# vt-asaplab/porla

Measured on AMD Instinct MI355X. Metric: BN254 G1 MSM Mscalar-mul/s at 2^20 pts, higher is better.
Workload: dtype u32x8 (256-bit modular integer); 1 GPU; KZG scheme, single 2^20-point BN254 G1 MSM per GPU, inputs resident in HBM, output 64-B affine point; pairs_per_gpu=1048576, msm_in_flight=2, warmup_steps_run=41, collective=none (single GPU)

## Files before the change

porla_amd/csrc/ec30.hip.h:

```cpp
#pragma once
#include "ec.hip.h"
#include "fe30.hip.h"

namespace porla {

template <class M>
struct XYZZ30 {
    F30<M> x, y, zz, zzz;
    bool inf;
};

template <class M>
__device__ __forceinline__ XYZZ<M> xyzz30_to_xyzz(const XYZZ30<M>& p);

template <class M>
__device__ __noinline__ XYZZ30<M> xyzz30_double_affine(F30<M> ax, F30<M> ay) {
    XYZZ30<M> r;
    F30<M> U = f30_small_mul<M, 2>(ay);
    F30<M> V = f30_sqr<M>(U);
    F30<M> W = f30_mul<M>(U, V);
    F30<M> S = f30_mul<M>(ax, V);
    F30<M> XX = f30_sqr<M>(ax);
    F30<M> Mm = f30_small_mul<M, 3>(XX);
    F30<M> MM = f30_sqr<M>(Mm);
// ... 210 lines not shown
    }
    xyzz30_add<M>(a, b);
    xyzz30_store_lazy<M>(p, a);
}
template <class M>
__device__ __noinline__ void xyzz30_double_mem(XYZZ<M>* p, int times) {
    XYZZ30<M> a = xyzz30_load_lazy<M>(p);
    if (a.inf) return;
#pragma unroll 1
    for (int t = 0; t < times && !a.inf; t++) a = xyzz30_double_body<M>(a.x, a.y, a.zz, a.zzz);
    xyzz30_store_lazy<M>(p, a);
}

template <int CTRL>
__device__ __forceinline__ uint32_t dpp_quad(uint32_t v) {
    return (uint32_t)__builtin_amdgcn_update_dpp(0, (int)v, CTRL, 0xf, 0xf, true);
}
template <class M, int CTRL>
__device__ __forceinline__ F30<M> f30_quad(const F30<M>& a) {
    F30<M> r;
#pragma unroll
    for (int i = 0; i < 9; i++) r.v[i] = dpp_quad<CTRL>(a.v[i]);
    return r;
}
template <class M>
__device__ __forceinline__ F30<M> f30_sel(bool c, const F30<M>& a, const F30<M>& b) {
    F30<M> r;
#pragma unroll
    for (int i = 0; i < 9; i++) r.v[i] = c ? a.v[i] : b.v[i];
    return r;
}
template <class M>
__device__ __forceinline__ F30<M> xyzz30_load_coord(const XYZZ<M>* p, int c, bool* all_zero) {
    const uint4* q = reinterpret_cast<const uint4*>(reinterpret_cast<const uint32_t*>(p) + 8 * c);
    const uint4 a = q[0], b = q[1];
    uint32_t t[8] = {a.x, a.y, a.z, a.w, b.x, b.y, b.z, b.w};
    *all_zero = (a.x | a.y | a.z | a.w | b.x | b.y | b.z | b.w) == 0;
    return f30_unpack<M>(t);
}
template <class M>
__device__ __forceinline__ void xyzz30_store_coord(XYZZ<M>* p, int c, const F30<M>& v, bool final) {
    uint32_t* d = reinterpret_cast<uint32_t*>(p) + 8 * c;
    Fe<M> t;
    if (final) {
        t = f30_to_fe_canonical<M>(f30_mul<M>(v, f30_const<M>(M::R1)));
    } else if constexpr (M::PSEUDO_MERSENNE) {
        t = f30_to_fe_canonical<M>(f30_pm_reduce<M>(v));
    } else {
        f30_pack<M>(t.v, v);
    }
    store_words8(d, t.v);
}
template <class M>
__device__ __noinline__ void xyzz30_add_one_lane(const XYZZ<M>* pa, const XYZZ<M>* pb, XYZZ<M>* out, bool final) {
    XYZZ30<M> a = xyzz30_load_lazy<M>(pa), b = xyzz30_load_lazy<M>(pb);
    xyzz30_add<M>(a, b);
    if (final) {
        const XYZZ<M> r = xyzz30_to_xyzz<M>(a);
        uint32_t* d = reinterpret_cast<uint32_t*>(out);
        store_words8(d, r.x.v); store_words8(d + 8, r.y.v); store_words8(d + 16, r.zz.v); store_words8(d + 24, r.zzz.v);
    } else {
        xyzz30_store_lazy<M>(out, a);
    }
}
template <class M>
__device__ __forceinline__ void xyzz30_add_quad(const XYZZ<M>* pa, const XYZZ<M>* pb, XYZZ<M>* out, bool final, bool live,
                                                uint32_t lane) {
    const uint32_t r = lane & 3u;
    const XYZZ<M>* sa = (r & 1u) ? pb : pa;
    const XYZZ<M>* sb = (r & 1u) ? pa : pb;
    bool za, zb;
    const F30<M> A = xyzz30_load_coord<M>(sa, (int)(r >> 1), &za);
    const F30<M> B = xyzz30_load_coord<M>(sb, 2 + (int)(r >> 1), &zb);
    bool special = zb;
    if (!final) {
        const uint32_t qz = (uint32_t)(__ballot(zb) >> (lane & 60u)) & 0xfu;
        if (qz) {
            const XYZZ<M>* src = (qz & 0x5u) ? pa : pb;
            if (live && src != out) {
                const uint4* q = reinterpret_cast<const uint4*>(reinterpret_cast<const uint32_t*>(src) + 8 * r);
                uint4* d = reinterpret_cast<uint4*>(reinterpret_cast<uint32_t*>(out) + 8 * r);
                const uint4 v0 = q[0], v1 = q[1];
                d[0] = v0; d[1] = v1;
            }
            return;
        }
    }
    const F30<M> M1 = f30_mul<M>(A, B);
    const bool edge = (r == 0u) || (r == 3u);
    const F30<M> rcv = f30_quad<M, 0xB1>(f30_sel<M>(edge, B, M1));
    const F30<M> D = f30_sub<M, 2>(f30_sel<M>(r == 0u, rcv, M1), f30_sel<M>(r == 0u, M1, rcv));
    const F30<M> M2 = f30_mul<M>(f30_sel<M>(edge, D, B), f30_sel<M>(edge, D, rcv));
    if (r == 0u && f30_product_is_zero<M>(M2)) special = true;
    const unsigned long long bal = __ballot(special);
    if ((bal >> (lane & 60u)) & 0xfull) {
        if (r == 0u && live) xyzz30_add_one_lane<M>(pa, pb, out, final);
        return;
    }
    const F30<M> bPP = f30_quad<M, 0x00>(M2);
    const F30<M> bU1 = f30_quad<M, 0x00>(M1);
    const F30<M> M3 = f30_mul<M>(r == 0u ? D : (r == 3u ? bU1 : M2), r == 0u ? M2 : bPP);
    const F30<M> bPPP = f30_quad<M, 0x00>(M3);
    const F30<M> bS1 = f30_quad<M, 0xAA>(M1);
    const F30<M> E = f30_add2<M>(bPPP, M3);
    const F30<M> X3 = f30_sub<M, 4>(M2, E);
    const F30<M> Dq = f30_sub<M, 6>(M3, X3);
    const F30<M> M4 = f30_mul<M>(r == 0u ? bS1 : (r == 3u ? D : M2), r == 3u ? Dq : bPPP);
    const F30<M> bT2 = f30_quad<M, 0x00>(M4);
    const F30<M> Y3 = f30_sub<M, 2>(M4, bT2);
    if (!live) return;
    if (r == 3u) { xyzz30_store_coord<M>(out, 0, X3, final); xyzz30_store_coord<M>(out, 1, Y3, final); }
    else if (r == 1u) xyzz30_store_coord<M>(out, 2, M3, final);
    else if (r == 2u) xyzz30_store_coord<M>(out, 3, M4, final);
}

template <class M>
__device__ __forceinline__ void xyzz30_dbl_quad(const XYZZ<M>* p, XYZZ<M>* out, bool live, uint32_t lane) {
    const uint32_t r = lane & 3u;
    bool zero;
    const F30<M> A = xyzz30_load_coord<M>(p, (int)r, &zero);
    const uint32_t qz = (uint32_t)(__ballot(zero && r == 2u) >> (lane & 60u)) & 0xfu;
    if (qz) {
        if (live && out != p) {
            uint4* d = reinterpret_cast<uint4*>(reinterpret_cast<uint32_t*>(out) + 8 * r);
            d[0] = make_uint4(0, 0, 0, 0); d[1] = d[0];
        }
        return;
    }
    const F30<M> U = f30_small_mul<M, 2>(A);
    const F30<M> O1 = f30_sel<M>(r == 1u, U, A);
    const F30<M> M1 = f30_mul<M>(O1, O1);
    const F30<M> bV = f30_quad<M, 0x55>(M1);
    const F30<M> bXX = f30_quad<M, 0x00>(M1);
    const F30<M> Mm = f30_small_mul<M, 3>(bXX);
    const F30<M> M2 = f30_mul<M>(r == 3u ? Mm : O1, r == 3u ? Mm : bV);
    const F30<M> bW = f30_quad<M, 0x55>(M2);
    const F30<M> bMM = f30_quad<M, 0xFF>(M2);
    const F30<M> S2 = f30_small_mul<M, 2>(M2);
    const F30<M> X3 = f30_sub<M, 3>(bMM, S2);
    const F30<M> D = f30_sub<M, 5>(M2, X3);
    const F30<M> M3 = f30_mul<M>(r == 0u ? Mm : bW, r == 0u ? D : A);
    const F30<M> bT2 = f30_quad<M, 0x55>(M3);
    const F30<M> Y3 = f30_sub<M, 2>(M3, bT2);
    if (!live) return;
    if (r == 0u) { xyzz30_store_coord<M>(out, 0, X3, false); xyzz30_store_coord<M>(out, 1, Y3, false); }
    else if (r == 2u) xyzz30_store_coord<M>(out, 2, M2, false);
    else if (r == 3u) xyzz30_store_coord<M>(out, 3, M3, false);
}

// ... 79 lines not shown
```

porla_amd/csrc/engine.hpp:

```cpp
#pragma once
#include <hip/hip_runtime.h>
#include <cstddef>
#include <cstdint>
#include <mutex>
#include <string>
#include <utility>
#include <vector>
#include "../../include/porla_gpu.h"
#include "host_curve.hpp"
#include "msm.hip.h"
#include "msm_small.hip.h"

namespace porla {

void set_last_error(const std::string& s);
int hip_fail(hipError_t e, const char* what, const char* file, int line);

#define PORLA_HIP(call)                                                      \
    do {                                                                     \
        hipError_t _e = (call);                                              \
        if (_e != hipSuccess) return ::porla::hip_fail(_e, #call, __FILE__, __LINE__); \
    } while (0)

struct ProfScope {
// ... 122 lines not shown
    void release() {
        if (h) retired.emplace_back(h, upload);
        for (auto& rb : retired) {
            if (rb.second) {
                (void)hipEventSynchronize(rb.second);
                (void)hipEventDestroy(rb.second);
            }
            (void)hipHostFree(rb.first);
        }
        retired.clear();
        h = nullptr;
        cap = 0;
        upload = nullptr;
    }
};

struct Workspace {
    std::mutex mu;
    int device = -1;
    Buf pts, keys, entries, counts, starts, fill, cursor, buckets, in_scalars, in_points;
    Buf order, blk_hist, blk_off, tile_off, heavy, chunk_out;
    Buf small_part;
    uint32_t small_seq = 0;
    Buf tree_s, tree_m, tree_mt;
    Buf multi_acc;
    hipEvent_t merged = nullptr;
    void* h_windows = nullptr;
    size_t h_windows_cap = 0;
    hipStream_t own_stream = nullptr;
    hipStream_t aux_stream = nullptr;
    hipEvent_t fork_ev = nullptr, join_ev = nullptr;
    hipEvent_t front_fork_ev = nullptr, front_join_ev = nullptr;
    hipEvent_t caller_ev = nullptr;
    int slot = 0;
    hipEvent_t done = nullptr;
    int pend_W = 0, pend_c = 0;
    bool lone = false;
    bool pair_pending = false;
    bool begun = false;
    Buf batch_list, batch_part, batch_sums, batch_ctrl, batch_out;
    PinnedList batch_list_h;
    UseFence batch_fence;
};
constexpr int MSM_SLOTS = 17;
constexpr int MSM_POOL_SLOTS = 8;
constexpr int MSM_AUDIT_SLOT = 16;
constexpr int MSM_USER_SLOTS = 4;
constexpr int MSM_MULTI_SLOT0 = 4;
constexpr int MSM_MULTI_SLOTS = 4;
constexpr int MSM_POOL_SLOT0 = 8;
int order_after_caller(Workspace* ws, hipStream_t caller, hipStream_t a, hipStream_t b = nullptr);
constexpr size_t MSM_SCAN_MAX = 1u << 16;
constexpr size_t MSM_RANGE_MAX = 1u << 22;
template <class C>
struct FixedBase {
    int device = -1;
    int c = 0, W = 0;
    size_t n_points = 0;
    Affine<typename C::Fp>* table = nullptr;
    size_t table_cap = 0;
    XYZZ<typename C::Fp>* pow_buf = nullptr;
    size_t pow_cap = 0;
    XYZZ<typename C::Fp>* scratch_buf = nullptr;
    size_t scratch_cap = 0;
    bool keep_build_buffers = false;
    XYZZ<typename C::Fp>* partial = nullptr;
    size_t partial_cap = 0;
    uint8_t* io_rows = nullptr;
    size_t io_rows_cap = 0;
    uint8_t* io_out = nullptr;
    size_t io_out_cap = 0;
    hipStream_t io_stream2 = nullptr;
    uint32_t last_S = 1;
    UseFence fence;
    static constexpr size_t HOST_FINISH_MAX_ROWS = 256;
    void* h_small = nullptr;
    void* d_small = nullptr;
    uint32_t small_seq = 0;
    hipEvent_t small_done = nullptr;
    std::mutex mu;
    void release();
    int build(const Affine<typename C::Fp>* d_base, size_t n, int window_bits, hipStream_t stream);
    int build_from_host_bytes(const uint8_t* points_be, size_t n, int window_bits, hipStream_t stream);
    int commit_device(const uint8_t* d_rows, size_t n_rows, size_t n_coeffs, size_t row_stride, uint8_t* d_out,
                      hipStream_t stream, bool guest_room = false);
    int commit_host(const uint8_t* rows, size_t n_rows, size_t n_coeffs, size_t row_stride, uint8_t* out,
                    hipStream_t stream);
    int commit_small(const uint8_t* const* row_ptrs, size_t n_rows, size_t n_coeffs, uint8_t* const* outs, hipStream_t stream,
                     const uint8_t* d_rows = nullptr, XYZZ<typename C::Fp>* raw_sums = nullptr);
    static bool small_ok(size_t n_rows, size_t n_coeffs);
};

}
struct porla_fixed_base {
    int curve;
    porla::FixedBase<porla::Bn254G1> bn;
    porla::FixedBase<porla::Secp256k1G> secp;
};
namespace porla {

extern std::mutex g_ws_mu;
extern int g_window_override;
extern int g_small_mode;
extern int g_small_c;
extern int g_last_multi[2];
extern int g_last_shape[3];
// ... 38 lines not shown
```

porla_amd/csrc/msm.hip.h:

```cpp
#pragma once
#include "ec.hip.h"
#include "ec30.hip.h"
#include "glv.hip.h"
#include <type_traits>

namespace porla {

struct Bn254G1 {
    using Fp = Bn254Fp;
    static constexpr uint32_t ORDER[8] = {0xf0000001u, 0x43e1f593u, 0x79b97091u, 0x2833e848u,
                                          0x8181585du, 0xb85045b6u, 0xe131a029u, 0x30644e72u};
    static constexpr int SCALAR_BITS = 254;
    static constexpr int MAX_Q = 5;
    using Glv = GlvBn254;
    static constexpr bool GLV_DEFAULT = false;
    static constexpr size_t GLV_BELOW = (size_t)1 << 17;
    static constexpr bool F30_BUCKETS = true;
    static constexpr bool F30_LAZY = true;
    static constexpr int BUCKET_SUM_WAVES = 4;
    static constexpr int FB_COMMIT_WAVES = 3;
    static constexpr int MACQ_WAVES = 4;
};
struct Secp256k1G {
    using Fp = Secp256k1Fp;
    static constexpr uint32_t ORDER[8] = {0xd0364141u, 0xbfd25e8cu, 0xaf48a03bu, 0xbaaedce6u,
                                          0xfffffffeu, 0xffffffffu, 0xffffffffu, 0xffffffffu};
    static constexpr int SCALAR_BITS = 256;
    static constexpr int MAX_Q = 1;
    using Glv = GlvSecp256k1;
    static constexpr bool GLV_DEFAULT = true;
    static constexpr size_t GLV_BELOW = 0;
    static constexpr bool F30_BUCKETS = true;
    static constexpr bool F30_LAZY = true;
    static constexpr int BUCKET_SUM_WAVES = 3;
    static constexpr int FB_COMMIT_WAVES = 2;
    static constexpr int MACQ_WAVES = 2;
};

constexpr uint32_t KEY_NONE = 0xffffffffu;

__device__ __forceinline__ void load_be256(uint32_t t[8], const uint8_t* p) {
    const uint4* q = reinterpret_cast<const uint4*>(p);
    uint4 hi = q[0], lo = q[1];
    t[7] = __builtin_bswap32(hi.x); t[6] = __builtin_bswap32(hi.y);
    t[5] = __builtin_bswap32(hi.z); t[4] = __builtin_bswap32(hi.w);
    t[3] = __builtin_bswap32(lo.x); t[2] = __builtin_bswap32(lo.y);
    t[1] = __builtin_bswap32(lo.z); t[0] = __builtin_bswap32(lo.w);
}
__device__ __forceinline__ void store_be256(uint8_t* p, const uint32_t t[8]) {
    uint4 hi, lo;
    hi.x = __builtin_bswap32(t[7]); hi.y = __builtin_bswap32(t[6]);
    hi.z = __builtin_bswap32(t[5]); hi.w = __builtin_bswap32(t[4]);
    lo.x = __builtin_bswap32(t[3]); lo.y = __builtin_bswap32(t[2]);
    lo.z = __builtin_bswap32(t[1]); lo.w = __builtin_bswap32(t[0]);
    uint4* q = reinterpret_cast<uint4*>(p);
    q[0] = hi; q[1] = lo;
}

template <class M>
__device__ __forceinline__ Affine<M> load_affine(const Affine<M>* pts, uint32_t idx) {
    const uint4* q = reinterpret_cast<const uint4*>(pts + idx);
    uint4 a = q[0], b = q[1], c = q[2], d = q[3];
    Affine<M> r;
    r.x.v[0] = a.x; r.x.v[1] = a.y; r.x.v[2] = a.z; r.x.v[3] = a.w;
    r.x.v[4] = b.x; r.x.v[5] = b.y; r.x.v[6] = b.z; r.x.v[7] = b.w;
    r.y.v[0] = c.x; r.y.v[1] = c.y; r.y.v[2] = c.z; r.y.v[3] = c.w;
    r.y.v[4] = d.x; r.y.v[5] = d.y; r.y.v[6] = d.z; r.y.v[7] = d.w;
    return r;
}
template <class M>
__device__ __forceinline__ void store_fe(uint32_t* dst, const Fe<M>& f) {
    uint4* q = reinterpret_cast<uint4*>(dst);
    q[0] = make_uint4(f.v[0], f.v[1], f.v[2], f.v[3]);
    q[1] = make_uint4(f.v[4], f.v[5], f.v[6], f.v[7]);
}
template <class M>
__device__ __forceinline__ Fe<M> load_fe(const uint32_t* src) {
    const uint4* q = reinterpret_cast<const uint4*>(src);
    uint4 a = q[0], b = q[1];
    Fe<M> f;
    f.v[0] = a.x; f.v[1] = a.y; f.v[2] = a.z; f.v[3] = a.w;
    f.v[4] = b.x; f.v[5] = b.y; f.v[6] = b.z; f.v[7] = b.w;
    return f;
}
template <class M>
__device__ __forceinline__ void store_xyzz(XYZZ<M>* dst, const XYZZ<M>& p) {
    uint32_t* d = reinterpret_cast<uint32_t*>(dst);
// ... 89 lines not shown
    const size_t n_sub = glv ? 2 * n : n;
    pl.tile_cap = glv ? 2 * TILE : TILE;
    pl.T_tiles = (uint32_t)((n + TILE - 1) / TILE);
    pl.lowbits = sort_lowbits(c, n_sub, W);
    pl.sort_half = false;
    {
        const int lb2 = pl.lowbits - 1, parts_log = c - 1 - lb2;
        if (lb2 >= 0 && lb2 <= 11 && parts_log <= 7 && (n_sub >> parts_log) <= 16384 && (pl.tile_cap >> parts_log) >= 64) {
            pl.lowbits = lb2;
            pl.sort_half = true;
        }
    }
    pl.P = 1 << (c - 1 - pl.lowbits);
    pl.wg = pl.T_tiles < 256 ? 256u / pl.T_tiles : 1u;
    if (pl.wg > 16) pl.wg = 16;
    if (pl.wg > (unsigned)W) pl.wg = (unsigned)W;
    return pl;
}
constexpr int SORT_HOLD_TILES = 16;
static inline bool sort_holds_runs(const SortFrontPlan& pl) { return pl.T_tiles <= 16u * SORT_HOLD_TILES; }

__device__ __forceinline__ uint32_t block_scan_1024(uint32_t v, uint32_t* wsum , uint32_t* total) {
    const uint32_t lane = threadIdx.x & 63, wv = threadIdx.x >> 6;
    uint32_t incl = v;
#pragma unroll
    for (int d = 1; d < 64; d <<= 1) {
        uint32_t o = __shfl_up(incl, d, 64);
        if (lane >= (uint32_t)d) incl += o;
    }
    if (lane == 63) wsum[wv] = incl;
    __syncthreads();
    uint32_t base = 0, tot = 0;
#pragma unroll
    for (int k = 0; k < 16; k++) {
        uint32_t s = wsum[k];
        if ((uint32_t)k < wv) base += s;
        tot += s;
    }
    __syncthreads();
    *total = tot;
    return base + incl - v;
}

template <class C, bool GLV>
__global__ void __launch_bounds__(TILE_THREADS)
k_digits_partition(const uint8_t* __restrict__ scalars, uint32_t n, int c, int W, int lowbits,
                   uint32_t* __restrict__ tile_items, uint16_t* __restrict__ tile_off, uint32_t* __restrict__ ctrl) {
    constexpr int SUBS = GLV ? 2 : 1;
    constexpr int LIMBS = GLV ? 4 : 8;
    constexpr int NSUB = TILE_SPT * SUBS;
    __shared__ uint32_t hist[MAX_PARTS];
    __shared__ uint32_t cursor[MAX_PARTS];
    __shared__ uint32_t stage[TILE * SUBS];
    const uint32_t tile = blockIdx.x, T = gridDim.x, tid = threadIdx.x;
    if (tile == 0 && blockIdx.y == 0 && tid < 4 + 128) ctrl[tid] = 0;
    const int P = 1 << (c - 1 - lowbits);
    const uint32_t B = 1u << (c - 1);
    const uint32_t mask = (1u << c) - 1;
    uint32_t t[NSUB][LIMBS];
    bool valid[TILE_SPT];
    uint32_t sneg = 0;
#pragma unroll
    for (int j = 0; j < TILE_SPT; j++) {
        uint32_t i = tile * TILE + j * TILE_THREADS + tid;
        valid[j] = i < n;
        uint32_t k[8];
#pragma unroll
        for (int q = 0; q < 8; q++) k[q] = 0;
        if (valid[j]) {
            load_be256(k, scalars + (size_t)i * 32);
            for (int q = 0; q < C::MAX_Q; q++) {
                uint32_t s[8];
                uint32_t br = 0;
#pragma unroll
                for (int q2 = 0; q2 < 8; q2++) s[q2] = sbb32(k[q2], C::ORDER[q2], br);
                if (br) break;
#pragma unroll
                for (int q2 = 0; q2 < 8; q2++) k[q2] = s[q2];
            }
        }
        if (GLV) {
            uint32_t m1[4], m2[4];
            bool n1, n2;
            glv_split<typename C::Glv>(k, m1, n1, m2, n2);
#pragma unroll
            for (int q = 0; q < 4; q++) { t[j * SUBS][q] = m1[q]; t[j * SUBS + (SUBS - 1)][q] = m2[q]; }
            sneg |= (n1 ? 1u : 0u) << (j * SUBS);
            sneg |= (n2 ? 1u : 0u) << (j * SUBS + (SUBS - 1));
        } else {
#pragma unroll
            for (int q = 0; q < LIMBS; q++) t[j][q] = k[q];
        }
    }
    uint32_t carry = 0;

    const bool shared_tile = gridDim.y > 1;
    for (int w = 0; w < W; w++) {
        const bool mine = !shared_tile || (uint32_t)w % gridDim.y == blockIdx.y;
        if (mine) {
            if (tid < MAX_PARTS) hist[tid] = 0;
            __syncthreads();
        }
        uint32_t key[NSUB];
        const int lo = w * c;
        const int limb = lo >> 5, sh = lo & 31;
        uint32_t wa[NSUB], wb[NSUB];
// ... 32 lines not shown
            if (mine && key[u] != KEY_NONE) {
                key[u] |= (dneg ^ ((sneg >> u) & 1u)) << 31;
                atomicAdd(&hist[(key[u] & 0x7fffffffu) & (uint32_t)(P - 1)], 1u);
            }
        }
        if (!mine) continue;
        __syncthreads();
        uint32_t pv = 0, pincl = 0;
        if (tid < MAX_PARTS) {
            pv = (tid < (uint32_t)P) ? hist[tid] : 0;
            pincl = pv;
#pragma unroll
            for (int d = 1; d < 64; d <<= 1) {
                const uint32_t o = __shfl_up(pincl, d, 64);
                if ((tid & 63u) >= (uint32_t)d) pincl += o;
            }
            if (tid == 63) cursor[0] = pincl;
        }
        __syncthreads();
        uint16_t* off = tile_off + ((size_t)w * T + tile) * (MAX_PARTS + 1);
        if (tid < MAX_PARTS) {
            const uint32_t excl = (tid >= 64 ? cursor[0] : 0u) + pincl - pv;
            off[tid] = (uint16_t)excl;
            hist[tid] = excl;
            if (tid == MAX_PARTS - 1) { off[MAX_PARTS] = (uint16_t)(excl + pv); cursor[1] = excl + pv; }
        }
        __syncthreads();
        const uint32_t total = cursor[1];
#pragma unroll
        for (int u = 0; u < NSUB; u++) {
            if (key[u] != KEY_NONE) {
                uint32_t bkt = key[u] & 0x7fffffffu;
                uint32_t pos = atomicAdd(&hist[bkt & (uint32_t)(P - 1)], 1u);
                uint32_t local = (uint32_t)((u / SUBS) * TILE_THREADS + tid) * SUBS + (u % SUBS);
                stage[pos] = (bkt >> (c - 1 - lowbits)) | ((key[u] >> 31) << lowbits) | (local << (lowbits + 1));
            }
        }
        __syncthreads();
        uint32_t* dst = tile_items + ((size_t)w * T + tile) * (TILE * SUBS);
        for (uint32_t i = tid; i < total; i += TILE_THREADS) dst[i] = stage[i];
        __syncthreads();
    }
}

template <int STAGE_CAP, int MAX_LOW, bool HOLD>
__global__ void __launch_bounds__(1024)
k_partition_sort(const uint32_t* __restrict__ tile_items, const uint16_t* __restrict__ tile_off, uint32_t T, uint32_t tile_cap,
                 int c, int lowbits, uint32_t* __restrict__ counts, uint32_t* __restrict__ starts,
                 uint32_t* __restrict__ entries, uint32_t* __restrict__ cursor) {
    __shared__ uint32_t cnt[MAX_LOW];
    __shared__ uint32_t stage[STAGE_CAP];
    __shared__ uint32_t wsum[16];
    __shared__ uint32_t base_sh, total_sh;
    const int P = 1 << (c - 1 - lowbits);
    const uint32_t nlow = 1u << lowbits;
    const uint32_t w = blockIdx.x / P, p = blockIdx.x % P;
    const uint32_t tid = threadIdx.x, lane = tid & 63;
    const uint32_t wv = HOLD ? (uint32_t)__builtin_amdgcn_readfirstlane((int)(tid >> 6)) : tid >> 6;
    const uint32_t lowmask = nlow - 1;
    for (uint32_t i = tid; i < nlow; i += 1024) cnt[i] = 0;
    __syncthreads();
    auto run_bounds = [&](uint32_t t, uint32_t& lo, uint32_t& hi) {
        lo = 0; hi = 0;
        if (t < T) {
            const uint16_t* off = tile_off + ((size_t)w * T + t) * (MAX_PARTS + 1);
            lo = off[p];
            hi = (p + 1 < (uint32_t)P) ? off[p + 1] : off[MAX_PARTS];
        }
    };
    auto run_items = [&](uint32_t t, uint32_t lo, uint32_t hi, uint32_t& a, uint32_t& b) {
        a = 0; b = 0;
        if (t < T) {
            const uint32_t* it = tile_items + ((size_t)w * T + t) * tile_cap;
            if (lo + lane < hi) a = it[lo + lane];
            if (lo + 64 + lane < hi) b = it[lo + 64 + lane];
        }
    };
    auto count_chunk = [&](bool active, uint32_t item) {
        const uint32_t low = active ? (item & lowmask) : 0xffffffffu;
        const uint32_t first = (uint32_t)__builtin_amdgcn_readfirstlane((int)low);
        const unsigned long long same = __ballot(low == first);
        if (__popcll(same) >= 8) {
            if (lane == (uint32_t)(__ffsll((long long)same) - 1)) atomicAdd(&cnt[first], (uint32_t)__popcll(same));
            if (active && low != first) atomicAdd(&cnt[low], 1u);
        } else if (active) {
            atomicAdd(&cnt[low], 1u);
        }
    };
    constexpr int D = HOLD ? SORT_HOLD_TILES : 1;
    constexpr uint32_t HELD_NONE = 0xffffffffu;
    uint32_t held_a[D], held_b[D];
    uint32_t bounds = 0;
    unsigned long long long_runs = 0;
    auto beyond_held = [&](auto&& chunk) {
        for (unsigned long long m = long_runs; m; m &= m - 1) {
            const int k = __ffsll((long long)m) - 1;
            const uint32_t lohi = (uint32_t)__builtin_amdgcn_readlane((int)bounds, k), hi = lohi >> 16, t = wv + 16 * (uint32_t)k;
            const uint32_t* it = tile_items + ((size_t)w * T + t) * tile_cap;
            for (uint32_t i0 = (lohi & 0xffffu) + 128; i0 < hi; i0 += 64) {
                const bool active = i0 + lane < hi;
                chunk(t, active, active ? it[i0 + lane] : 0u);
            }
        }
    };
    if constexpr (HOLD) {
        if (lane < (uint32_t)D) {
// ... 91 lines not shown
            if (__ballot(held_b[k] != HELD_NONE)) place_chunk(wv + 16 * k, held_b[k] != HELD_NONE, held_b[k]);
        }
        beyond_held(place_chunk);
    } else {
        uint32_t lo1, hi1, lo2, hi2, a1, b1;
        run_bounds(wv, lo1, hi1);
        run_bounds(wv + 16, lo2, hi2);
        run_items(wv, lo1, hi1, a1, b1);
        for (uint32_t t = wv; t < T; t += 16) {
            const uint32_t lo = lo1, hi = hi1, a = a1, b = b1;
            lo1 = lo2; hi1 = hi2;
            run_bounds(t + 32, lo2, hi2);
            run_items(t + 16, lo1, hi1, a1, b1);
            const uint32_t* it = tile_items + ((size_t)w * T + t) * tile_cap;
            for (uint32_t i0 = lo; i0 < hi; i0 += 64) {
                const bool active = i0 + lane < hi;
                const uint32_t item = i0 == lo ? a : (i0 == lo + 64 ? b : (active ? it[i0 + lane] : 0u));
                place_chunk(t, active, item);
            }
        }
    }
    if (staged) {
        __syncthreads();
        for (uint32_t i = tid; i < total_sh; i += 1024) entries[base_sh + i] = stage[i];
    }
}

static inline void sort_launch(const SortFrontPlan& pl, int c, int W, hipStream_t stream, const uint32_t* tile_items, const uint16_t* tile_off,
                               uint32_t* counts, uint32_t* starts, uint32_t* entries, uint32_t* cursor) {
    const dim3 grid((unsigned)(W * pl.P)), block(1024);
    auto go = [&](auto kernel) {
        hipLaunchKernelGGL(kernel, grid, block, 0, stream, tile_items, tile_off, pl.T_tiles, pl.tile_cap, c, pl.lowbits, counts, starts, entries,
                           cursor);
    };
    const bool hold = sort_holds_runs(pl);
    if (pl.sort_half) {
        if (hold) go(k_partition_sort<SORT_STAGE_CAP / 2, SORT_MAX_LOW / 2, true>);
        else go(k_partition_sort<SORT_STAGE_CAP / 2, SORT_MAX_LOW / 2, false>);
    } else {
        if (hold) go(k_partition_sort<SORT_STAGE_CAP, SORT_MAX_LOW, true>);
        else go(k_partition_sort<SORT_STAGE_CAP, SORT_MAX_LOW, false>);
    }
}

constexpr int CHUNK = 128;
constexpr int CTRL_WORDS = 4 + CHUNK;
static_assert(CTRL_WORDS == 4 + 128, "k_digits_partition clears the control words");
constexpr uint32_t NO_CHUNK = 0xffffffffu;

static __global__ void __launch_bounds__(1024)
k_size_hist(const uint32_t* __restrict__ counts, uint32_t nb, uint32_t* __restrict__ blk_hist, uint32_t nblocks,
            uint32_t* __restrict__ ctrl) {
    __shared__ uint32_t hist[CHUNK];
    if (threadIdx.x < CHUNK) hist[threadIdx.x] = 0;
    __syncthreads();
    uint32_t i = blockIdx.x * blockDim.x + threadIdx.x;
    if (i < nb) {
        uint32_t cnt = counts[i];
        uint32_t full = cnt / CHUNK, rem = cnt % CHUNK;
        if (full) atomicAdd(&hist[0], full);
        if (rem) atomicAdd(&hist[CHUNK - rem], 1u);
    }
    __syncthreads();
    if (threadIdx.x < CHUNK) {
        uint32_t v = hist[threadIdx.x];
        blk_hist[(size_t)threadIdx.x * nblocks + blockIdx.x] = v;
    }
}

static __global__ void __launch_bounds__(1024)
k_size_scan(const uint32_t* __restrict__ blk_hist, uint32_t* __restrict__ blk_off, uint32_t nblocks,
            uint32_t* __restrict__ ctrl) {
    __shared__ uint32_t wsum[16];
    const uint32_t row = blockIdx.x, tid = threadIdx.x;
    uint32_t run = 0;
    for (uint32_t b0 = 0; b0 < nblocks; b0 += 1024) {
        uint32_t x = (b0 + tid < nblocks) ? blk_hist[(size_t)row * nblocks + b0 + tid] : 0;
        uint32_t tot;
        uint32_t e = block_scan_1024(x, wsum, &tot);
        if (b0 + tid < nblocks) blk_off[(size_t)row * nblocks + b0 + tid] = run + e;
        run += tot;
        __syncthreads();
    }
    if (tid == 0) ctrl[4 + row] = run;
}

static __global__ void __launch_bounds__(1024)
k_size_order(const uint32_t* __restrict__ counts, uint32_t nb, const uint32_t* __restrict__ blk_off, uint32_t nblocks,
             uint2* __restrict__ order, uint32_t* __restrict__ chunk_base, uint32_t* __restrict__ heavy_list,
             uint32_t* __restrict__ ctrl, uint4* __restrict__ buckets_raw) {
    __shared__ uint32_t next[CHUNK];
    __shared__ uint32_t wsum[16];
    {
        uint32_t total;
        const uint32_t v = (threadIdx.x < CHUNK) ? ctrl[4 + threadIdx.x] : 0;
        const uint32_t excl = block_scan_1024(v, wsum, &total);
        if (threadIdx.x < CHUNK) next[threadIdx.x] = excl + blk_off[(size_t)threadIdx.x * nblocks + blockIdx.x];
        if (blockIdx.x == 0 && threadIdx.x == 0) ctrl[3] = total;
    }
    __syncthreads();
    uint32_t i = blockIdx.x * blockDim.x + threadIdx.x;
    if (i >= nb) return;
    uint32_t cnt = counts[i];
    uint32_t full = cnt / CHUNK, rem = cnt % CHUNK;
    uint32_t items = full + (rem ? 1u : 0u);
    if (items == 0 && buckets_raw) {
        uint4 z = make_uint4(0, 0, 0, 0);
        uint4* d = buckets_raw + (size_t)i * 8;
#pragma unroll
        for (int k = 0; k < 8; k++) d[k] = z;
    }
    if (full) {
        uint32_t pos = atomicAdd(&next[0], full);
        for (uint32_t j = 0; j < full; j++) order[pos + j] = make_uint2(i, j);
    }
    if (rem) {
        uint32_t pos = atomicAdd(&next[CHUNK - rem], 1u);
        order[pos] = make_uint2(i, full);
    }
    if (items > 1) {
        chunk_base[i] = atomicAdd(&ctrl[1], items);
        heavy_list[atomicAdd(&ctrl[2], 1u)] = i;
    } else {
        chunk_base[i] = NO_CHUNK;
    }
}

template <class C>
__global__ void __launch_bounds__(256) __attribute__((amdgpu_waves_per_eu(C::BUCKET_SUM_WAVES, 4)))
k_bucket_sum30(const Affine<typename C::Fp>* __restrict__ pts, const uint32_t* __restrict__ entries,
               const uint32_t* __restrict__ starts, const uint32_t* __restrict__ counts,
               const uint2* __restrict__ order, const uint32_t* __restrict__ chunk_base,
               const uint32_t* __restrict__ ctrl, XYZZ<typename C::Fp>* __restrict__ buckets,
               XYZZ<typename C::Fp>* __restrict__ chunk_out, uint32_t accumulate) {
    using M = typename C::Fp;
    uint32_t tid = blockIdx.x * blockDim.x + threadIdx.x;
    if (tid >= ctrl[3]) return;
    uint2 item = order[tid];
    const uint32_t b = item.x;
    const uint32_t first = item.y * CHUNK;
    uint32_t cnt = counts[b] - first;
    if (cnt > CHUNK) cnt = CHUNK;
    const uint32_t* e = entries + starts[b] + first;
    const uint32_t cb = chunk_base[b];
    XYZZ30<M> acc = xyzz30_infinity<M>();
    if constexpr (C::F30_LAZY) {
        if (accumulate && cb == NO_CHUNK) acc = xyzz30_load_lazy<M>(buckets + b);
    }
    bool flip = false;
    uint32_t ent = e[0];
    uint32_t k = 0;
    if (acc.inf) {
        const uint32_t cur = ent;
        if (cnt > 1) ent = e[1];
        Affine<M> a = load_affine<M>(pts, cur & 0x7fffffffu);
        if (!aff_is_inf<M>(a)) {
            a = aff_neg_if<M>(a, (cur >> 31) != 0);
            acc.x = f30_from_fe<M>(a.x); acc.y = f30_from_fe<M>(a.y);
            acc.zz = f30_const<M>(M::R1_30); acc.zzz = acc.zz;
            acc.inf = false;
        }
        k = 1;
        if (!acc.inf && cnt > 1) {
            const uint32_t cur2 = ent;
            uint32_t nxt = cur2;
            if (cnt > 2) nxt = e[2];
            Affine<M> a2 = load_affine<M>(pts, cur2 & 0x7fffffffu);
            const bool a2_inf = aff_is_inf<M>(a2);
            a2 = aff_neg_if<M>(a2, xyzz30_flip_neg<M>((cur2 >> 31) != 0, flip));
            if (xyzz30_mmadd_flip_fast<M>(acc, flip, f30_from_fe<M>(a2.x), f30_from_fe<M>(a2.y), a2_inf)) { ent = nxt; k = 2; }
        }
    }
    {
        for (; k < cnt; k++) {
            const uint32_t cur = ent;
            uint32_t nxt = cur;
            if (k + 1 < cnt) nxt = e[k + 1];
            Affine<M> a = load_affine<M>(pts, cur & 0x7fffffffu);
            const bool a_inf = aff_is_inf<M>(a);
            a = aff_neg_if<M>(a, xyzz30_flip_neg<M>((cur >> 31) != 0, flip));
// ... 56 lines not shown
        else xyzz_add_cold<M>(&a, &b);
    }
    static __device__ __forceinline__ void store(XYZZ<M>* p, const T& a) {
        if constexpr (C::F30_LAZY) xyzz30_store_lazy<M>(p, a);
        else store_xyzz<M>(p, a);
    }
    static __device__ __forceinline__ void store_final(XYZZ<M>* p, const T& a) {
        if constexpr (C::F30_LAZY) store_xyzz<M>(p, xyzz30_to_xyzz<M>(a));
        else store_xyzz<M>(p, a);
    }
    static __device__ __forceinline__ T inf() {
        if constexpr (C::F30_LAZY) { T r; r.x = r.y = r.zz = r.zzz = F30<M>{}; r.inf = true; return r; }
        else return xyzz_inf<M>();
    }
};

template <class M>
struct TreeOp {
    const XYZZ<M>*pa, *pb;
    XYZZ<M>* out;
    bool final;
    bool copy;
};
template <class M>
__device__ __forceinline__ TreeOp<M> tree_op(const TreeLevelArgs<M>& a, uint32_t s, uint32_t i, uint32_t jp, uint32_t jo) {
    TreeOp<M> o;
    o.final = a.last != 0;
    o.copy = (s == a.l + 1);
    if (o.copy) {
        o.pa = a.s_prev + 2 * (size_t)i + 1; o.pb = o.pa;
        o.out = a.fin + (size_t)i * (a.nlev + 1) + 1 + a.l;
        return o;
    }
    if (s == a.l) { o.pa = a.s_prev + 2 * (size_t)i; o.pb = o.pa + 1; }
    else if (s + 1 == a.l) { o.pa = a.s_prev2 + 4 * (size_t)i + 1; o.pb = o.pa + 2; }
    else { o.pa = a.m_prev + (size_t)s * a.m_prev_stride + 2 * (size_t)jp; o.pb = o.pa + 1; }
    if (a.last) o.out = a.fin + (size_t)i * (a.nlev + 1) + (s == a.l ? 0 : 1 + s);
    else o.out = (s == a.l) ? a.s_out + i : a.m_out + (size_t)s * a.m_out_stride + jo;
    return o;
}
template <class C>
__device__ __forceinline__ void tree_task(const TreeLevelArgs<typename C::Fp>& a, uint32_t s, uint32_t i, uint32_t jp, uint32_t jo) {
    using M = typename C::Fp;
    using N = Node<C>;
    const TreeOp<M> o = tree_op<M>(a, s, i, jp, jo);
    typename N::T x = N::load(o.pa);
    if (!o.copy) {
        typename N::T y = N::load(o.pb);
        N::add(x, y);
    }
    if (o.final) N::store_final(o.out, x);
    else N::store(o.out, x);
}
template <class C>
__device__ __forceinline__ void tree_task_quad(const TreeLevelArgs<typename C::Fp>& a, uint32_t s, uint32_t i, uint32_t jp, uint32_t jo,
                                               bool live, uint32_t lane) {
    using M = typename C::Fp;
    const TreeOp<M> o = tree_op<M>(a, s, i, jp, jo);
    if (o.copy) {
        if (live && (lane & 3u) == 0u) Node<C>::store_final(o.out, Node<C>::load(o.pa));
        return;
    }
    xyzz30_add_quad<M>(o.pa, o.pb, o.out, o.final, live, lane);
}

template <class C>
__global__ void __launch_bounds__(256)
k_tree_level(TreeLevelArgs<typename C::Fp> a) {
    uint32_t t = blockIdx.x * blockDim.x + threadIdx.x;
    uint32_t slots = a.l + 1 + a.last;
    if (t >= slots * a.n) return;
    const uint32_t i = t % a.n;
    tree_task<C>(a, t / a.n, i, i, i);
}

template <class C>
__global__ void __launch_bounds__(256)
k_tree_level_quad(TreeLevelArgs<typename C::Fp> a) {
    const uint32_t tid = blockIdx.x * blockDim.x + threadIdx.x;
    const uint32_t total = (a.l + 1 + a.last) * a.n;
    uint32_t t = tid >> 2;
    const bool live = t < total;
    if (!live) t = total - 1;
    const uint32_t i = t % a.n;
    tree_task_quad<C>(a, t / a.n, i, i, i, live, threadIdx.x & 63u);
}

template <class C>
__global__ void __launch_bounds__(256)
k_tree_front2(TreeLevelArgs<typename C::Fp> a, XYZZ<typename C::Fp>* __restrict__ s1_out) {
    using M = typename C::Fp;
    using N = Node<C>;
    const uint32_t i = blockIdx.x * blockDim.x + threadIdx.x;
    if (i >= a.n) return;
    const XYZZ<M>* bk = a.s_prev + 4 * (size_t)i;
    typename N::T x = N::inf(), y = N::inf(), keep = N::inf();
#pragma unroll 1
    for (uint32_t s = 0; s < 4; s++) {
        if (s == 0) { x = N::load(bk); y = N::load(bk + 1); }
        else if (s == 1) { x = y; y = N::load(bk + 3); }
        else if (s == 2) { x = N::load(bk + 2); }
        else { y = x; x = keep; }
        N::add(x, y);
        if (s == 0) keep = x;
        else N::store(s == 1 ? a.m_out + i : (s == 2 ? a.s_out + 2 * (size_t)i + 1 : s1_out + i), x);
    }
}

template <class M>
struct TreeTailArgs {
    const XYZZ<M>* buckets;
    XYZZ<M>* s_lev[24];
    const XYZZ<M>* m_global;
    XYZZ<M>* m_tail[2];
    XYZZ<M>* fin;
    uint32_t nb;
    uint32_t B;
    uint32_t per_window;
    uint32_t l0;
    uint32_t nlev;
};
template <class C, bool QUAD>
__global__ void __launch_bounds__(512)
k_tree_tail(TreeTailArgs<typename C::Fp> a) {
    using M = typename C::Fp;
    const uint32_t w = blockIdx.x;
    for (uint32_t l = a.l0; l < a.nlev; l++) {
        const uint32_t nw = a.B >> (l + 1);
        TreeLevelArgs<M> lv;
        lv.s_prev = l ? a.s_lev[l - 1] : a.buckets;
        lv.s_prev2 = l >= 2 ? a.s_lev[l - 2] : a.buckets;
        lv.n = a.nb >> (l + 1);
        const bool first = (l == a.l0);
        lv.m_prev = first ? a.m_global : a.m_tail[(l + 1) & 1] + (size_t)w * a.per_window;
        lv.m_prev_stride = first ? 2 * lv.n : 2 * nw;
        lv.s_out = a.s_lev[l];
        lv.m_out = a.m_tail[l & 1] + (size_t)w * a.per_window;
        lv.m_out_stride = nw;
        lv.fin = a.fin;
        lv.l = l;
        lv.nlev = a.nlev;
        lv.last = (l + 1 == a.nlev) ? 1u : 0u;
        const uint32_t tasks = (l + 1 + lv.last) * nw;
        if constexpr (QUAD) {
            const uint32_t per_pass = blockDim.x >> 2;
            for (uint32_t t0 = 0; t0 < tasks; t0 += per_pass) {
                uint32_t t = t0 + (threadIdx.x >> 2);
                const bool live = t < tasks;
                if (!live) t = tasks - 1;
                const uint32_t j = t % nw, i = w * nw + j;
                tree_task_quad<C>(lv, t / nw, i, first ? i : j, j, live, threadIdx.x & 63u);
            }
        } else {
            for (uint32_t t = threadIdx.x; t < tasks; t += blockDim.x) {
                const uint32_t j = t % nw, i = w * nw + j;
                tree_task<C>(lv, t / nw, i, first ? i : j, j);
            }
        }
        __threadfence();
        __syncthreads();
    }
}

template <class C>
__global__ void __launch_bounds__(64)
k_bucket_combine(const uint32_t* __restrict__ heavy_list, const uint32_t* __restrict__ chunk_base,
                 const uint32_t* __restrict__ counts, const uint32_t* __restrict__ ctrl,
                 const XYZZ<typename C::Fp>* __restrict__ chunk_out, XYZZ<typename C::Fp>* __restrict__ buckets,
                 uint32_t accumulate) {
    using M = typename C::Fp;
    using N = Node<C>;
    __shared__ XYZZ<M> stage[64];
    const uint32_t n_heavy = ctrl[2];
    for (uint32_t h = blockIdx.x; h < n_heavy; h += gridDim.x) {
        const uint32_t b = heavy_list[h];
        const uint32_t items = (counts[b] + CHUNK - 1) / CHUNK;
        const XYZZ<M>* src = chunk_out + chunk_base[b];
        typename N::T acc = N::inf();
        if (accumulate && threadIdx.x == 0) acc = N::load(buckets + b);
        for (uint32_t k = threadIdx.x; k < items; k += 64) {
            typename N::T p = N::load(src + k);
            N::add(acc, p);
        }
        for (uint32_t m = 32; m >= 1; m >>= 1) {
            N::store(&stage[threadIdx.x], acc);
            __syncthreads();
            if (threadIdx.x < m) {
                typename N::T o = N::load(&stage[threadIdx.x + m]);
                N::add(acc, o);
            }
            __syncthreads();
        }
        if (threadIdx.x == 0) N::store(buckets + b, acc);
    }
}

}
```

porla_amd/csrc/msm_impl.hip.h:

```cpp
#pragma once
#include "engine.hpp"
#include "host_fold64.hpp"
#include "msm_small.hip.h"
#include "msm_tree.hip.h"
#include <cstdlib>
#include <chrono>
#include <thread>
#include <vector>
#include <cstdio>
#include "../../include/porla_gpu.h"

namespace porla {

static inline int ilog2(size_t n) { int l = 0; while (n >>= 1) l++; return l; }

constexpr double TREE_US_PER_ADD = 1.5e-4;
constexpr double TREE_LEVEL_US = 12.5;
constexpr double TREE_QUAD_LEVEL_US = 7.0;
constexpr double TREE_TAIL_LEVEL_US = 6.5;
static inline int choose_window(size_t m, int bits) {
    if (g_window_override >= 2 && g_window_override <= 20) return g_window_override;
    int best = 2;
    double best_cost = 1e300;
    for (int c = 2; c <= 20; c++) {
// ... 208 lines not shown
    uint32_t* ctrl = (uint32_t*)ws->cursor.p;
    const Affine<M>* pts = (const Affine<M>*)ws->pts.p;
    const bool front_split = ws->lone && !forced && n >= ((size_t)1 << 18);
    hipStream_t pst = stream;
    if (front_split) {
        if (!ws->aux_stream) PORLA_HIP(hipStreamCreateWithFlags(&ws->aux_stream, hipStreamNonBlocking));
        if (!ws->front_fork_ev) PORLA_HIP(hipEventCreateWithFlags(&ws->front_fork_ev, hipEventDisableTiming));
        if (!ws->front_join_ev) PORLA_HIP(hipEventCreateWithFlags(&ws->front_join_ev, hipEventDisableTiming));
        PORLA_HIP(hipEventRecord(ws->front_fork_ev, stream));
        PORLA_HIP(hipStreamWaitEvent(ws->aux_stream, ws->front_fork_ev, 0));
        pst = ws->aux_stream;
    }
    {
        ProfScope ps("points_to_mont", pst);
        if (glv)
            hipLaunchKernelGGL((k_points_to_mont<C, true, C::F30_BUCKETS>), dim3((n32 + 255) / 256), dim3(256), 0, pst, d_points_be,
                               (Affine<M>*)ws->pts.p, n32);
        else
            hipLaunchKernelGGL((k_points_to_mont<C, false, C::F30_BUCKETS>), dim3((n32 + 255) / 256), dim3(256), 0, pst, d_points_be,
                               (Affine<M>*)ws->pts.p, n32);
    }
    if (front_split) PORLA_HIP(hipEventRecord(ws->front_join_ev, ws->aux_stream));
    {
        ProfScope ps("digits_partition", stream);
        if (glv)
            hipLaunchKernelGGL((k_digits_partition<C, true>), dim3(T_tiles, sf.wg), dim3(TILE_THREADS), 0, stream, d_scalars, n32, c, W,
                               lowbits, (uint32_t*)ws->keys.p, (uint16_t*)ws->tile_off.p, ctrl);
        else
            hipLaunchKernelGGL((k_digits_partition<C, false>), dim3(T_tiles, sf.wg), dim3(TILE_THREADS), 0, stream, d_scalars, n32, c, W,
                               lowbits, (uint32_t*)ws->keys.p, (uint16_t*)ws->tile_off.p, ctrl);
    }
    {
        ProfScope ps("partition_sort", stream);
        sort_launch(sf, c, W, stream, (const uint32_t*)ws->keys.p, (const uint16_t*)ws->tile_off.p, (uint32_t*)ws->counts.p,
                    (uint32_t*)ws->starts.p, (uint32_t*)ws->entries.p, ctrl);
    }
    {
        ProfScope ps("size_order", stream);
        hipLaunchKernelGGL(k_size_hist, dim3(nblk), dim3(1024), 0, stream, (const uint32_t*)ws->counts.p, (uint32_t)nb,
                           (uint32_t*)ws->blk_hist.p, nblk, ctrl);
        hipLaunchKernelGGL(k_size_scan, dim3(CHUNK), dim3(1024), 0, stream, (const uint32_t*)ws->blk_hist.p,
                           (uint32_t*)ws->blk_off.p, nblk, ctrl);
        hipLaunchKernelGGL(k_size_order, dim3(nblk), dim3(1024), 0, stream, (const uint32_t*)ws->counts.p, (uint32_t)nb,
                           (const uint32_t*)ws->blk_off.p, nblk, (uint2*)ws->order.p, (uint32_t*)ws->fill.p,
                           (uint32_t*)ws->heavy.p, ctrl, accumulate ? (uint4*)nullptr : (uint4*)bk);
    }
    if (accumulate) {
        if (!C::F30_LAZY) { set_last_error("porla: merged pair ranges need the reduced-radix bucket form"); return PORLA_ERR_STATE; }
        if (after) PORLA_HIP(hipStreamWaitEvent(stream, after, 0));
    }
    if (front_split) PORLA_HIP(hipStreamWaitEvent(stream, ws->front_join_ev, 0));
    {
        ProfScope ps("bucket_sum", stream, true);
        hipLaunchKernelGGL((k_bucket_sum30<C>), dim3((unsigned)((max_items + 255) / 256)), dim3(256), 0, stream, pts,
                           (const uint32_t*)ws->entries.p, (const uint32_t*)ws->starts.p,
                           (const uint32_t*)ws->counts.p, (const uint2*)ws->order.p, (const uint32_t*)ws->fill.p,
                           (const uint32_t*)ctrl, bk, (XYZZ<M>*)ws->chunk_out.p, accumulate ? 1u : 0u);
    }
    {
        ProfScope ps("bucket_combine", stream);
        hipLaunchKernelGGL((k_bucket_combine<C>), dim3(2048), dim3(64), 0, stream, (const uint32_t*)ws->heavy.p,
                           (const uint32_t*)ws->fill.p, (const uint32_t*)ws->counts.p, (const uint32_t*)ctrl,
                           (const XYZZ<M>*)ws->chunk_out.p, bk, accumulate ? 1u : 0u);
    }
    PORLA_HIP(hipGetLastError());
    if (forced) return PORLA_OK;
    return msm_tree_launch<C>(ws, bk, c, W, glv, stream);
}

template <class C>
static int msm_tree_launch(Workspace* ws, const XYZZ<typename C::Fp>* buckets, int c, int W, bool glv, hipStream_t stream) {
    using M = typename C::Fp;
    int rc;
    static thread_local TreePlan plan;
    static thread_local int plan_c = 0, plan_W = 0, plan_lone = -1;
    if (plan_c != c || plan_W != W || plan_lone != (ws->lone ? 1 : 0)) {
        plan_c = 0;
        const std::string refused = tree_plan(plan, c, W, ws->lone, C::F30_LAZY);
        if (!refused.empty()) { set_last_error("porla: reduction tree: " + refused); return PORLA_ERR_STATE; }
        plan_c = c; plan_W = W; plan_lone = ws->lone ? 1 : 0;
    }
    if ((rc = ws->tree_s.ensure(plan.s_entries * sizeof(XYZZ<M>)))) return rc;
    if ((rc = ws->tree_m.ensure(plan.m_entries * sizeof(XYZZ<M>)))) return rc;
    if ((rc = ws->tree_mt.ensure(plan.mt_entries * sizeof(XYZZ<M>)))) return rc;
    if (ws->h_windows_cap < (size_t)W * c * sizeof(XYZZ<M>) || ws->h_windows_cap < 64 * 1024) {
        if (ws->h_windows) PORLA_HIP(hipHostFree(ws->h_windows));
        ws->h_windows_cap = 64 * 1024;
        PORLA_HIP(hipHostMalloc(&ws->h_windows, ws->h_windows_cap, hipHostMallocMapped | hipHostMallocCoherent));
    }
    void* h_windows_dev = nullptr;
    PORLA_HIP(hipHostGetDevicePointer(&h_windows_dev, ws->h_windows, 0));
    const int parts = (int)plan.parts;
    if (parts == 2) {
        if (!ws->aux_stream) PORLA_HIP(hipStreamCreateWithFlags(&ws->aux_stream, hipStreamNonBlocking));
        if (!ws->fork_ev) PORLA_HIP(hipEventCreateWithFlags(&ws->fork_ev, hipEventDisableTiming));
        if (!ws->join_ev) PORLA_HIP(hipEventCreateWithFlags(&ws->join_ev, hipEventDisableTiming));
        PORLA_HIP(hipEventRecord(ws->fork_ev, stream));
        PORLA_HIP(hipStreamWaitEvent(ws->aux_stream, ws->fork_ev, 0));
    }
    PORLA_HIP((tree_enqueue<C, ProfScope>(plan, buckets, (XYZZ<M>*)ws->tree_s.p, (XYZZ<M>*)ws->tree_m.p, (XYZZ<M>*)ws->tree_mt.p,
                                          (XYZZ<M>*)h_windows_dev, stream, ws->aux_stream)));
    if (parts == 2) {
        PORLA_HIP(hipEventRecord(ws->join_ev, ws->aux_stream));
        PORLA_HIP(hipStreamWaitEvent(stream, ws->join_ev, 0));
    }
    if (!ws->done) PORLA_HIP(hipEventCreateWithFlags(&ws->done, hipEventDisableTiming));
    PORLA_HIP(hipEventRecord(ws->done, stream));
// ... 408 lines not shown
```

Measured before the change: 796.6 Mmul/s.

## Co-schedule BN254 tree kernels as high-priority guests beside bucket sum

For BN254, the front-end sort and tree kernels now raise their wave priority. The tree kernels are pinned to a fixed waves-per-EU occupancy, and bucket_sum is launched with dummy dynamic LDS to cap its occupancy, so that a concurrent MSM's tree and front stages can fit alongside it on the CUs. The cold one-lane fallback is inlined in the level-quad kernel and given a separate noinline copy in the tail. bucket_combine is rewritten to accumulate in LDS through the noinline one-lane add, which cuts register pressure. This trades lower bucket_sum occupancy and extra LDS traffic for better overlap between the two in-flight MSMs.

```diff
diff --git a/porla_amd/csrc/ec30.hip.h b/porla_amd/csrc/ec30.hip.h
--- a/porla_amd/csrc/ec30.hip.h
+++ b/porla_amd/csrc/ec30.hip.h
@@ -286,7 +286,7 @@
     store_words8(d, t.v);
 }
 template <class M>
-__device__ __noinline__ void xyzz30_add_one_lane(const XYZZ<M>* pa, const XYZZ<M>* pb, XYZZ<M>* out, bool final) {
+__device__ __forceinline__ void xyzz30_add_one_lane_body(const XYZZ<M>* pa, const XYZZ<M>* pb, XYZZ<M>* out, bool final) {
     XYZZ30<M> a = xyzz30_load_lazy<M>(pa), b = xyzz30_load_lazy<M>(pb);
     xyzz30_add<M>(a, b);
     if (final) {
@@ -298,6 +298,14 @@
     }
 }
 template <class M>
+__device__ __noinline__ void xyzz30_add_one_lane(const XYZZ<M>* pa, const XYZZ<M>* pb, XYZZ<M>* out, bool final) {
+    xyzz30_add_one_lane_body<M>(pa, pb, out, final);
+}
+template <class M>
+static __device__ __noinline__ void xyzz30_add_one_lane_guest(const XYZZ<M>* pa, const XYZZ<M>* pb, XYZZ<M>* out, bool final) {
+    xyzz30_add_one_lane_body<M>(pa, pb, out, final);
+}
+template <class M, int COLD = 0>
 __device__ __forceinline__ void xyzz30_add_quad(const XYZZ<M>* pa, const XYZZ<M>* pb, XYZZ<M>* out, bool final, bool live,
                                                 uint32_t lane) {
     const uint32_t r = lane & 3u;
@@ -328,7 +336,11 @@
     if (r == 0u && f30_product_is_zero<M>(M2)) special = true;
     const unsigned long long bal = __ballot(special);
     if ((bal >> (lane & 60u)) & 0xfull) {
-        if (r == 0u && live) xyzz30_add_one_lane<M>(pa, pb, out, final);
+        if (r == 0u && live) {
+            if constexpr (COLD == 1) xyzz30_add_one_lane_body<M>(pa, pb, out, final);
+            else if constexpr (COLD == 2) xyzz30_add_one_lane_guest<M>(pa, pb, out, final);
+            else xyzz30_add_one_lane<M>(pa, pb, out, final);
+        }
         return;
     }
     const F30<M> bPP = f30_quad<M, 0x00>(M2);
diff --git a/porla_amd/csrc/engine.hpp b/porla_amd/csrc/engine.hpp
--- a/porla_amd/csrc/engine.hpp
+++ b/porla_amd/csrc/engine.hpp
@@ -198,6 +198,7 @@
 int order_after_caller(Workspace* ws, hipStream_t caller, hipStream_t a, hipStream_t b = nullptr);
 constexpr size_t MSM_SCAN_MAX = 1u << 16;
 constexpr size_t MSM_RANGE_MAX = 1u << 22;
+constexpr size_t MSM_GUEST_MIN_PAIRS = 1u << 17;
 template <class C>
 struct FixedBase {
     int device = -1;
diff --git a/porla_amd/csrc/msm.hip.h b/porla_amd/csrc/msm.hip.h
--- a/porla_amd/csrc/msm.hip.h
+++ b/porla_amd/csrc/msm.hip.h
@@ -18,6 +18,8 @@
     static constexpr bool F30_BUCKETS = true;
     static constexpr bool F30_LAZY = true;
     static constexpr int BUCKET_SUM_WAVES = 4;
+    static constexpr bool TREE_GUEST = true;
+    static constexpr int TREE_WAVES_MIN = TREE_GUEST ? 4 : 1, TREE_WAVES_MAX = TREE_GUEST ? 4 : 8;
     static constexpr int FB_COMMIT_WAVES = 3;
     static constexpr int MACQ_WAVES = 4;
 };
@@ -33,6 +35,8 @@
     static constexpr bool F30_BUCKETS = true;
     static constexpr bool F30_LAZY = true;
     static constexpr int BUCKET_SUM_WAVES = 3;
+    static constexpr bool TREE_GUEST = false;
+    static constexpr int TREE_WAVES_MIN = 1, TREE_WAVES_MAX = 8;
     static constexpr int FB_COMMIT_WAVES = 2;
     static constexpr int MACQ_WAVES = 2;
 };
@@ -228,6 +232,7 @@
     __shared__ uint32_t hist[MAX_PARTS];
     __shared__ uint32_t cursor[MAX_PARTS];
     __shared__ uint32_t stage[TILE * SUBS];
+    __builtin_amdgcn_s_setprio(3);
     const uint32_t tile = blockIdx.x, T = gridDim.x, tid = threadIdx.x;
     if (tile == 0 && blockIdx.y == 0 && tid < 4 + 128) ctrl[tid] = 0;
     const int P = 1 << (c - 1 - lowbits);
@@ -366,6 +371,7 @@
     __shared__ uint32_t stage[STAGE_CAP];
     __shared__ uint32_t wsum[16];
     __shared__ uint32_t base_sh, total_sh;
+    __builtin_amdgcn_s_setprio(3);
     const int P = 1 << (c - 1 - lowbits);
     const uint32_t nlow = 1u << lowbits;
     const uint32_t w = blockIdx.x / P, p = blockIdx.x % P;
@@ -563,6 +569,7 @@
 k_size_hist(const uint32_t* __restrict__ counts, uint32_t nb, uint32_t* __restrict__ blk_hist, uint32_t nblocks,
             uint32_t* __restrict__ ctrl) {
     __shared__ uint32_t hist[CHUNK];
+    __builtin_amdgcn_s_setprio(3);
     if (threadIdx.x < CHUNK) hist[threadIdx.x] = 0;
     __syncthreads();
     uint32_t i = blockIdx.x * blockDim.x + threadIdx.x;
@@ -583,6 +590,7 @@
 k_size_scan(const uint32_t* __restrict__ blk_hist, uint32_t* __restrict__ blk_off, uint32_t nblocks,
             uint32_t* __restrict__ ctrl) {
     __shared__ uint32_t wsum[16];
+    __builtin_amdgcn_s_setprio(3);
     const uint32_t row = blockIdx.x, tid = threadIdx.x;
     uint32_t run = 0;
     for (uint32_t b0 = 0; b0 < nblocks; b0 += 1024) {
@@ -602,6 +610,7 @@
              uint32_t* __restrict__ ctrl, uint4* __restrict__ buckets_raw) {
     __shared__ uint32_t next[CHUNK];
     __shared__ uint32_t wsum[16];
+    __builtin_amdgcn_s_setprio(3);
     {
         uint32_t total;
         const uint32_t v = (threadIdx.x < CHUNK) ? ctrl[4 + threadIdx.x] : 0;
@@ -637,6 +646,7 @@
     }
 }
 
+constexpr unsigned BUCKET_SUM_GUEST_LDS = 41 * 1024;
 template <class C>
 __global__ void __launch_bounds__(256) __attribute__((amdgpu_waves_per_eu(C::BUCKET_SUM_WAVES, 4)))
 k_bucket_sum30(const Affine<typename C::Fp>* __restrict__ pts, const uint32_t* __restrict__ entries,
@@ -799,7 +809,7 @@
     if (o.final) N::store_final(o.out, x);
     else N::store(o.out, x);
 }
-template <class C>
+template <class C, int COLD = 0>
 __device__ __forceinline__ void tree_task_quad(const TreeLevelArgs<typename C::Fp>& a, uint32_t s, uint32_t i, uint32_t jp, uint32_t jo,
                                                bool live, uint32_t lane) {
     using M = typename C::Fp;
@@ -808,12 +818,15 @@
         if (live && (lane & 3u) == 0u) Node<C>::store_final(o.out, Node<C>::load(o.pa));
         return;
     }
-    xyzz30_add_quad<M>(o.pa, o.pb, o.out, o.final, live, lane);
-}
+    xyzz30_add_quad<M, COLD>(o.pa, o.pb, o.out, o.final, live, lane);
+}
+
+#define MSM_TREE_GUEST_ATTR __attribute__((amdgpu_waves_per_eu(C::TREE_WAVES_MIN, C::TREE_WAVES_MAX)))
 
 template <class C>
-__global__ void __launch_bounds__(256)
+__global__ void __launch_bounds__(256) MSM_TREE_GUEST_ATTR
 k_tree_level(TreeLevelArgs<typename C::Fp> a) {
+    if constexpr (C::TREE_GUEST) __builtin_amdgcn_s_setprio(3);
     uint32_t t = blockIdx.x * blockDim.x + threadIdx.x;
     uint32_t slots = a.l + 1 + a.last;
     if (t >= slots * a.n) return;
@@ -822,15 +835,16 @@
 }
 
 template <class C>
-__global__ void __launch_bounds__(256)
+__global__ void __launch_bounds__(256) MSM_TREE_GUEST_ATTR
 k_tree_level_quad(TreeLevelArgs<typename C::Fp> a) {
+    if constexpr (C::TREE_GUEST) __builtin_amdgcn_s_setprio(3);
     const uint32_t tid = blockIdx.x * blockDim.x + threadIdx.x;
     const uint32_t total = (a.l + 1 + a.last) * a.n;
     uint32_t t = tid >> 2;
     const bool live = t < total;
     if (!live) t = total - 1;
     const uint32_t i = t % a.n;
-    tree_task_quad<C>(a, t / a.n, i, i, i, live, threadIdx.x & 63u);
+    tree_task_quad<C, C::TREE_GUEST ? 1 : 0>(a, t / a.n, i, i, i, live, threadIdx.x & 63u);
 }
 
 template <class C>
@@ -868,9 +882,10 @@
     uint32_t nlev;
 };
 template <class C, bool QUAD>
-__global__ void __launch_bounds__(512)
+__global__ void __launch_bounds__(512) MSM_TREE_GUEST_ATTR
 k_tree_tail(TreeTailArgs<typename C::Fp> a) {
     using M = typename C::Fp;
+    if constexpr (C::TREE_GUEST) __builtin_amdgcn_s_setprio(3);
     const uint32_t w = blockIdx.x;
     for (uint32_t l = a.l0; l < a.nlev; l++) {
         const uint32_t nw = a.B >> (l + 1);
@@ -896,7 +911,7 @@
                 const bool live = t < tasks;
                 if (!live) t = tasks - 1;
                 const uint32_t j = t % nw, i = w * nw + j;
-                tree_task_quad<C>(lv, t / nw, i, first ? i : j, j, live, threadIdx.x & 63u);
+                tree_task_quad<C, C::TREE_GUEST ? 2 : 0>(lv, t / nw, i, first ? i : j, j, live, threadIdx.x & 63u);
             }
         } else {
             for (uint32_t t = threadIdx.x; t < tasks; t += blockDim.x) {
@@ -910,7 +925,7 @@
 }
 
 template <class C>
-__global__ void __launch_bounds__(64)
+__global__ void __launch_bounds__(64) MSM_TREE_GUEST_ATTR
 k_bucket_combine(const uint32_t* __restrict__ heavy_list, const uint32_t* __restrict__ chunk_base,
                  const uint32_t* __restrict__ counts, const uint32_t* __restrict__ ctrl,
                  const XYZZ<typename C::Fp>* __restrict__ chunk_out, XYZZ<typename C::Fp>* __restrict__ buckets,
@@ -918,17 +933,42 @@
     using M = typename C::Fp;
     using N = Node<C>;
     __shared__ XYZZ<M> stage[64];
+    if constexpr (C::TREE_GUEST) __builtin_amdgcn_s_setprio(3);
     const uint32_t n_heavy = ctrl[2];
     for (uint32_t h = blockIdx.x; h < n_heavy; h += gridDim.x) {
         const uint32_t b = heavy_list[h];
         const uint32_t items = (counts[b] + CHUNK - 1) / CHUNK;
         const XYZZ<M>* src = chunk_out + chunk_base[b];
+        if constexpr (C::TREE_GUEST) {
+            uint4* mine = reinterpret_cast<uint4*>(&stage[threadIdx.x]);
+            const uint4* seed = reinterpret_cast<const uint4*>(buckets + b);
+            const bool seeded = accumulate && threadIdx.x == 0;
+#pragma unroll
+            for (int i = 0; i < 8; i++) mine[i] = seeded ? seed[i] : make_uint4(0, 0, 0, 0);
+#pragma unroll 1
+            for (uint32_t k = threadIdx.x; k < items; k += 64)
+                xyzz30_add_one_lane_guest<M>(&stage[threadIdx.x], src + k, &stage[threadIdx.x], false);
+#pragma unroll 1
+            for (uint32_t m = 32; m >= 1; m >>= 1) {
+                __syncthreads();
+                if (threadIdx.x < m) xyzz30_add_one_lane_guest<M>(&stage[threadIdx.x], &stage[threadIdx.x + m], &stage[threadIdx.x], false);
+                __syncthreads();
+            }
+            if (threadIdx.x == 0) {
+                uint4* d = reinterpret_cast<uint4*>(buckets + b);
+#pragma unroll
+                for (int i = 0; i < 8; i++) d[i] = mine[i];
+            }
+            continue;
+        }
         typename N::T acc = N::inf();
         if (accumulate && threadIdx.x == 0) acc = N::load(buckets + b);
+#pragma unroll 1
         for (uint32_t k = threadIdx.x; k < items; k += 64) {
             typename N::T p = N::load(src + k);
             N::add(acc, p);
         }
+#pragma unroll 1
         for (uint32_t m = 32; m >= 1; m >>= 1) {
             N::store(&stage[threadIdx.x], acc);
             __syncthreads();
diff --git a/porla_amd/csrc/msm_impl.hip.h b/porla_amd/csrc/msm_impl.hip.h
--- a/porla_amd/csrc/msm_impl.hip.h
+++ b/porla_amd/csrc/msm_impl.hip.h
@@ -284,7 +284,8 @@
     if (front_split) PORLA_HIP(hipStreamWaitEvent(stream, ws->front_join_ev, 0));
     {
         ProfScope ps("bucket_sum", stream, true);
-        hipLaunchKernelGGL((k_bucket_sum30<C>), dim3((unsigned)((max_items + 255) / 256)), dim3(256), 0, stream, pts,
+        const bool guest = C::TREE_GUEST && !ws->lone && !forced && n >= MSM_GUEST_MIN_PAIRS;
+        hipLaunchKernelGGL((k_bucket_sum30<C>), dim3((unsigned)((max_items + 255) / 256)), dim3(256), guest ? BUCKET_SUM_GUEST_LDS : 0, stream, pts,
                            (const uint32_t*)ws->entries.p, (const uint32_t*)ws->starts.p,
                            (const uint32_t*)ws->counts.p, (const uint2*)ws->order.p, (const uint32_t*)ws->fill.p,
                            (const uint32_t*)ctrl, bk, (XYZZ<M>*)ws->chunk_out.p, accumulate ? 1u : 0u);
```

Measured after the change: 830.7 Mmul/s, median of 6. +4.3%, better.
